# chkda/pytorch-distributed-tutorials

Hardware: AMD Instinct MI355X
Metric: images/sec (whole node) ResNet-50 bf16 at 1/2/4/8 MI355X (higher is better)
Workload: dtype bf16; 1 GPU; model=resnet50, global_batch=256, image_size=224, parallelism=dp1, impl=native, backend=nccl, wire_dtype=fp32, comm_backend=auto, cudnn_benchmark=False, graph=False, deterministic=False, force_comm=False, plan_world=1

## Files before the change

build_native.py:

```python
#!/usr/bin/env python3
from __future__ import annotations

import argparse
import concurrent.futures as cf
import glob
import os
import shlex
import subprocess
import sys
import sysconfig

ROOT = os.path.dirname(os.path.abspath(__file__))
CSRC = os.path.join(ROOT, "csrc")
PKG = os.path.join(ROOT, "pytorch_distributed_tutorials_amd")
BUILD = os.path.join(ROOT, "build", "native")
ARCH = os.environ.get("PYTORCH_ROCM_ARCH", "gfx950").split(";")[0]
HIPCC = os.environ.get("HIPCC", "/opt/rocm/bin/hipcc")


def _torch_paths():
    import torch
    tdir = os.path.dirname(torch.__file__)
    inc = [os.path.join(tdir, "include"), os.path.join(tdir, "include", "torch", "csrc", "api", "include")]
    return tdir, inc, int(torch._C._GLIBCXX_USE_CXX11_ABI)
# ... 67 lines not shown
    os.makedirs(os.path.dirname(so), exist_ok=True)
    if force or jobs_list or not os.path.exists(so) or os.path.getmtime(so) < max(os.path.getmtime(o) for o in objs):
        tlib = os.path.join(tdir, "lib")
        link = [HIPCC, "-shared", "-fPIC", f"--offload-arch={ARCH}", "-o", so] + objs + [
            "-L", tlib, "-lc10", "-lc10_hip", "-ltorch", "-ltorch_cpu", "-ltorch_hip", "-ltorch_python",
            os.path.join(tlib, "librccl.so"), f"-Wl,-rpath,{tlib}", "-Wl,-rpath,/opt/rocm/lib"]
        if sanitize:
            link += ["-fsanitize=address,undefined", "-shared-libsan"]
        _run(link)
        if verbose:
            print(f"[build_native] linked {os.path.relpath(so, ROOT)}", flush=True)
    return so


def ensure_built(verbose: bool = False) -> str:
    return build(force=False, verbose=verbose)


def main(argv=None) -> int:
    ap = argparse.ArgumentParser(description=__doc__, formatter_class=argparse.RawDescriptionHelpFormatter)
    ap.add_argument("--force", action="store_true")
    ap.add_argument("--jobs", type=int, default=0)
    ap.add_argument("--debug", action="store_true")
    ap.add_argument("--sanitize", action="store_true", help="host ASan+UBSan build into build/asan/")
    a = ap.parse_args(argv)
    so = build(force=a.force, jobs=a.jobs, debug=a.debug, sanitize=a.sanitize)
    print(so)
    return 0


# ... 3 lines not shown
```

csrc/bindings.cpp:

```cpp
#include <ATen/ATen.h>
#include <c10/hip/HIPGuard.h>
#include <c10/hip/HIPCachingAllocator.h>
#include <c10/hip/HIPStream.h>
#include <torch/extension.h>

#include <cstdlib>
#include <optional>
#include <stdexcept>
#include <string>
#include <type_traits>
#include <unordered_map>

#include "comm/rccl_comm.h"
#include "comm/xgmi_comm.h"
#include "ddp/reducer.h"
#include "kernels/kernels.h"

namespace py = pybind11;
using at::Tensor;

namespace {

bool g_sync_check = [] {
  const char* e = std::getenv("PDT_SYNC_CHECK");
// ... 310 lines not shown
  TORCH_CHECK(stats.numel() == 4 * K && gamma.numel() == K && sums.numel() == 2 * K && sums.is_contiguous(),
              "BN operands: [4,K], [K], [2,K]");
  int* dp = nullptr;
  if (done.has_value() && done->defined()) {
    TORCH_CHECK(done->is_cuda() && done->scalar_type() == at::kInt && done->numel() >= C / 64 + 1,
                "done: int32 device counters [C / 64 + 1]");
    dp = done->data_ptr<int>();
  }
  TORCH_CHECK(!zero_sums || dp != nullptr, "zero_sums needs the completion counter");
  c10::hip::HIPGuard g(wt.get_device());
  auto pg = bn_param_sinks(dgamma, dbeta, K);
  pdt::launch_bn_fold_wgrad(t1.data_ptr<float>(), gram.data_ptr<float>(), colsum.data_ptr<float>(),
                            reinterpret_cast<const uint16_t*>(wt.data_ptr()), stats.data_ptr<float>(),
                            gamma.data_ptr<float>(), sums.data_ptr<float>(), (int)count, C, K, out.data_ptr<float>(),
                            pg.first, pg.second, dp, zero_sums, cur_stream(wt), csum_slots);
}

std::tuple<Tensor, Tensor> conv_dgrad_bn_fold(const Tensor& g, const Tensor& z_in, const Tensor& wfold,
                                              const Tensor& bias, const Tensor& y, const std::optional<Tensor>& z,
                                              const Tensor& stats, int64_t mask, const std::optional<Tensor>& acc,
                                              const std::optional<Tensor>& dgamma,
                                              const std::optional<Tensor>& dbeta) {
  check_bf16_nhwc(g, "g");
  check_bf16_nhwc(z_in, "z_in");
  const int K = g.size(3), C = z_in.size(3);
  TORCH_CHECK(z_in.size(0) == g.size(0) && z_in.size(1) == g.size(1) && z_in.size(2) == g.size(2),
              "fold: g and z must share N, H, W");
  TORCH_CHECK(wfold.scalar_type() == at::kBFloat16 && wfold.is_contiguous() && wfold.size(0) == C &&
              wfold.size(1) == K + C, "wfold must be bf16 [C][K + C]");
  TORCH_CHECK(bias.scalar_type() == at::kFloat && bias.numel() == C, "bias: fp32 [C]");
// ... 1143 lines not shown
  m.def("stem_bwd_fused", checked("stem_bwd_fused", &stem_bwd_fused), py::arg("dpool"), py::arg("idx"),
        py::arg("y"), py::arg("stats"), py::arg("gamma"), py::arg("sums"), py::arg("training"), py::arg("xsp"),
        py::arg("w_shape"), py::arg("deterministic") = false, py::arg("out") = py::none());
  m.def("stem_bwd_fused_supported", &pdt::stem_bwd_fused_supported, py::arg("K"), py::arg("R"), py::arg("Sp"),
        py::arg("Ho"), py::arg("Wo"));
  m.def("bn_finalize", checked("bn_finalize", &bn_finalize), py::arg("part"), py::arg("count"), py::arg("rm"),
        py::arg("rv"), py::arg("gamma"), py::arg("beta"), py::arg("momentum"), py::arg("eps"),
        py::arg("grows") = 0);
  m.def("bn_eval_params", checked("bn_eval_params", &bn_eval_params));
  m.def("bn_fold_weights", checked("bn_fold_weights", &bn_fold_weights), py::arg("wt"), py::arg("stats"),
        py::arg("gamma"), py::arg("sums"), py::arg("count"));
  m.def("bn_fold_wgrad", checked("bn_fold_wgrad", &bn_fold_wgrad), py::arg("t1"), py::arg("gram"),
        py::arg("colsum"), py::arg("wt"), py::arg("stats"), py::arg("gamma"), py::arg("sums"), py::arg("count"),
        py::arg("out"), py::arg("dgamma") = py::none(), py::arg("dbeta") = py::none(),
        py::arg("done") = py::none(), py::arg("zero_sums") = false);
  m.def("conv_dgrad_bn_fold", checked("conv_dgrad_bn_fold", &conv_dgrad_bn_fold), py::arg("g"), py::arg("z_in"),
        py::arg("wfold"), py::arg("bias"), py::arg("y"), py::arg("z"), py::arg("stats"), py::arg("mask"),
        py::arg("acc") = py::none(), py::arg("dgamma") = py::none(), py::arg("dbeta") = py::none());
  m.def("conv_fwd_bn", checked("conv_fwd_bn", &conv_fwd_bn), py::arg("x"), py::arg("wk"), py::arg("stride"),
        py::arg("pad"), py::arg("count"), py::arg("rm"), py::arg("rv"), py::arg("gamma"), py::arg("beta"),
        py::arg("momentum"), py::arg("eps"), py::arg("acc") = py::none());
  m.def("bn_act_fwd", checked("bn_act_fwd", &bn_act_fwd), py::arg("y"), py::arg("scale"), py::arg("shift"),
        py::arg("residual"), py::arg("relu"), py::arg("res_scale") = py::none(),
        py::arg("res_shift") = py::none(), py::arg("csum") = py::none());
  m.def("bn_act_fwd_mask", checked("bn_act_fwd_mask", &bn_act_fwd_mask), py::arg("y"), py::arg("scale"),
        py::arg("shift"), py::arg("residual"), py::arg("res_scale") = py::none(),
        py::arg("res_shift") = py::none());
  m.def("bn_act_bwd_reduce", checked("bn_act_bwd_reduce", &bn_act_bwd_reduce), py::arg("dz"), py::arg("z"), py::arg("y"),
        py::arg("stats"), py::arg("mask"), py::arg("dgamma") = py::none(), py::arg("dbeta") = py::none());
  m.def("bn_act_bwd_apply", checked("bn_act_bwd_apply", &bn_act_bwd_apply), py::arg("dz"), py::arg("z"),
// ... 91 lines not shown
  m.def("conv_wgrad_cu_reserve", &pdt::conv_wgrad_cu_reserve);
  m.def("conv_wgrad_plan", [](std::vector<int64_t> x_shape, std::vector<int64_t> w_shape, int stride, int pad,
                              bool deterministic) {
    TORCH_CHECK(x_shape.size() == 4 && w_shape.size() == 4, "x_shape [N,H,W,C], w_shape [K,C,R,S]");
    pdt::ConvShape s{};
    s.N = (int)x_shape[0]; s.H = (int)x_shape[1]; s.W = (int)x_shape[2]; s.C = (int)x_shape[3];
    s.K = (int)w_shape[0]; s.R = (int)w_shape[2]; s.S = (int)w_shape[3];
    s.stride = stride; s.pad = pad;
    s.Ho = (s.H + 2 * pad - s.R) / stride + 1; s.Wo = (s.W + 2 * pad - s.S) / stride + 1;
    int out[4];
    pdt::conv_wgrad_plan(s, deterministic, out);
    py::dict d;
    d["bm"] = out[0]; d["bn"] = out[1]; d["tiles"] = out[2]; d["splits"] = out[3];
    return d;
  }, py::arg("x_shape"), py::arg("w_shape"), py::arg("stride"), py::arg("pad"), py::arg("deterministic") = false);
  m.def("bn_counter_bank", [](uintptr_t stream) {
    return pdt::bn_counter_bank(reinterpret_cast<hipStream_t>(stream));
  }, py::arg("stream"));
  m.def("cu_masked_stream", [](int device, int ncu) {
    c10::hip::HIPGuard guard((c10::DeviceIndex)device);
    int total = 0;
    if (hipDeviceGetAttribute(&total, hipDeviceAttributeMultiprocessorCount, device) != hipSuccess || total <= 0)
      throw std::runtime_error("cu_masked_stream: cannot query the CU count");
    ncu = std::max(1, std::min(ncu, total));
    std::vector<uint32_t> mask((total + 31) / 32, 0u);
    for (int i = 0; i < ncu; ++i) {
      const int cu = (int)((int64_t)i * total / ncu);
      mask[cu / 32] |= 1u << (cu % 32);
    }
    hipStream_t s = nullptr;
// ... 114 lines not shown
```

csrc/kernels/bn_act.hip:

```cpp
#include "common.h"
#include "fp8_util.h"
#include "igemm_common.h"
#include "kernels.h"
#include "pool_quad.h"

#include <algorithm>
#include <cstdlib>
#include <mutex>
#include <numeric>
#include <stdexcept>
#include <unordered_map>

namespace pdt {

__device__ __forceinline__ void load8(const float* p, float (&v)[8]) {
  float4 a = *reinterpret_cast<const float4*>(p);
  float4 b = *reinterpret_cast<const float4*>(p + 4);
  v[0] = a.x; v[1] = a.y; v[2] = a.z; v[3] = a.w; v[4] = b.x; v[5] = b.y; v[6] = b.z; v[7] = b.w;
}

#ifndef PDT_FIN_CH
#define PDT_FIN_CH 32
#endif
constexpr int FIN_CH = PDT_FIN_CH;
// ... 216 lines not shown
    a = -k1 * k2;
    b = -k1 * (sums[k] * invM - mu * k2);
  }
};

constexpr int kFoldMaxK = 2048;
constexpr int kCsumSlots = 128, kCsumBlocks = 4096;
typedef __bf16 fold_v8bf __attribute__((ext_vector_type(8)));

__global__ void __launch_bounds__(256) bn_fold_coef_kernel(FoldCoef cf, float* __restrict__ coef) {
  __builtin_amdgcn_s_setprio(3);
  const int k = blockIdx.x * 256 + threadIdx.x;
  if (k < cf.K) cf.ab(k, coef[k], coef[cf.K + k]);
}

__global__ void __launch_bounds__(256) bn_fold_weights_kernel(const uint16_t* __restrict__ wt, FoldCoef cf,
                                                              const float* __restrict__ coef, int C, int nG,
                                                              uint16_t* __restrict__ wfold,
                                                              float* __restrict__ bias,
                                                              float* __restrict__ part) {
  __builtin_amdgcn_s_setprio(3);
  const int K = cf.K, t = threadIdx.x;
  const int KC = K + C;
  const int bid = blockIdx.x;
  if (bid >= nG) {
    const int64_t e = ((int64_t)(bid - nG) * 256 + t) * 8;
    if (e >= (int64_t)C * K) return;
    const int c = (int)(e / K), k = (int)(e - (int64_t)c * K);
    f8 v = unpack8(*reinterpret_cast<const uint4*>(wt + e));
    float g8[8], i8[8];
// ... 24 lines not shown
    xa[q] = *reinterpret_cast<const uint4*>(pa + q * 16);
    xb[q] = *reinterpret_cast<const uint4*>(pb + q * 16);
  }
  for (int k0 = 0; k0 < kq; k0 += 16 * B4) {
    const bool more = k0 + 16 * B4 < kq;
    if (more) {
#pragma unroll
      for (int q = 0; q < B4; ++q) {
        ya[q] = *reinterpret_cast<const uint4*>(pa + k0 + 16 * B4 + q * 16);
        yb[q] = *reinterpret_cast<const uint4*>(pb + k0 + 16 * B4 + q * 16);
      }
    }
#pragma unroll
    for (int q = 0; q < B4; ++q) {
      const int kb = k0 + q * 16;
      float a8[8];
      load8(ca_ + kb, a8);
      f8 fa = unpack8(xa[q]);
      if (with_bias) {
        float b8[8];
        load8(cb_ + kb, b8);
#pragma unroll
        for (int e = 0; e < 8; ++e) bacc = fmaf(fa.v[e], b8[e], bacc);
      }
#pragma unroll
      for (int e = 0; e < 8; ++e) fa.v[e] *= a8[e];
      const uint4 qa = pack8(fa);
      acc = __builtin_amdgcn_mfma_f32_32x32x16_bf16(__builtin_bit_cast(fold_v8bf, qa),
                                                    __builtin_bit_cast(fold_v8bf, xb[q]), acc, 0, 0, 0);
    }
    if (more) {
#pragma unroll
      for (int q = 0; q < B4; ++q) { xa[q] = ya[q]; xb[q] = yb[q]; }
    }
  }
  float* pw = part + (size_t)bid * (3 * 17 * 64);
// ... 130 lines not shown
}

void launch_bn_fold_wgrad(float* t1, float* gram, const float* colsum, const uint16_t* wt,
                          const float* stats, const float* gamma, const float* sums, int M, int C, int K,
                          float* out, float* dgamma, float* dbeta, int* done, bool zero_sums, hipStream_t st,
                          int csum_slots) {
  if (C % kFoldTile != 0 || K % kFoldTile != 0)
    throw std::runtime_error("bn_fold_wgrad: needs C % 64 == 0, K % 64 == 0");
  if (csum_slots != 1 && (csum_slots != kCsumSlots || done == nullptr))
    throw std::runtime_error("bn_fold_wgrad: column sums come as 1 vector, or bn_act_fwd's slots in consume mode");
  FoldCoef cf{stats, gamma, sums, K, 1.f / (float)M};
  hipLaunchKernelGGL(bn_fold_wgrad_kernel, dim3((K / kFoldTile) * (C / kFoldTile)), dim3(256), 0, st, t1, gram,
                     colsum, wt, cf, C, out, dgamma, dbeta, done, zero_sums ? 1 : 0, csum_slots);
}

int64_t bn_fold_weights_ws_floats(int C, int K) { return C + 2 * (int64_t)K + (int64_t)(C / 32) * (C / 32) * 3 * 17 * 64; }

void launch_bn_fold_weights(const uint16_t* wt, const float* stats, const float* gamma, const float* sums,
                            int M, int C, int K, uint16_t* wfold, float* bias, hipStream_t st) {
  if (C % 32 != 0 || K % 256 != 0 || K > kFoldMaxK)
    throw std::runtime_error("bn_fold_weights: needs C % 32 == 0, K % 256 == 0, K <= 2048");
  const int nG = (C / 32) * (C / 32);
  const int nS = (int)(((int64_t)C * K / 8 + 255) / 256);
  FoldCoef cf{stats, gamma, sums, K, 1.f / (float)M};
  float* coef = bias + C;
  float* part = coef + 2 * K;
  hipLaunchKernelGGL(bn_fold_coef_kernel, dim3(ceil_div(K, 256)), dim3(256), 0, st, cf, coef);
  hipLaunchKernelGGL(bn_fold_weights_kernel, dim3(nG + nS), dim3(256), 0, st, wt, cf, coef, C, nG, wfold, bias,
                     part);
}

__global__ void bn_eval_params_kernel(const float* rm, const float* rv, const float* gamma,
                                      const float* beta, float eps, int K, float* out) {
  int k = blockIdx.x * blockDim.x + threadIdx.x;
  if (k >= K) return;
  float invstd = rsqrtf(rv[k] + eps);
  float sc = gamma[k] * invstd;
  out[k] = rm[k];
  out[K + k] = invstd;
  out[2 * K + k] = sc;
  out[3 * K + k] = beta[k] - rm[k] * sc;
}

void launch_bn_eval_params(const float* rm, const float* rv, const float* gamma, const float* beta,
// ... 761 lines not shown
```

csrc/kernels/kernels.h:

```cpp
#pragma once
#include <hip/hip_runtime.h>
#include <stdint.h>

namespace pdt {

void launch_image_to_nhwc(const float* x, uint16_t* y, int N, int C, int H, int W, int Cp,
                          hipStream_t st);
void launch_pack_weight(const float* w, const int64_t* strides, uint16_t* out, int K, int C,
                        int R, int S, int Cp, hipStream_t st);
void launch_pack_t_batched(const uint16_t* src, uint16_t* dst, const void* table, int ntensors,
                           int max_tiles, hipStream_t st);
size_t pack_t_entry_bytes();
void launch_stem_image(const float* x, uint16_t* xsp, int N, int C, int H, int W, int pad, int Hp,
                       int Wsp, hipStream_t st);
bool stem_halo_supported(int K, int R, int Sp, int Wo);
void launch_stem_conv_fwd(const uint16_t* xsp, const uint16_t* wsp, uint16_t* y, float* part, int N, int Hp,
                          int Wsp, int Ho, int Wo, hipStream_t st);
bool stem_bwd_fused_supported(int K, int R, int Sp, int Ho, int Wo);
int stem_bwd_fused_blocks(int N, int Ho);
void launch_stem_bwd_fused(const uint16_t* dpool, const uint8_t* idx, const uint16_t* y, const float* stats,
                           const float* gamma, const float* sums, bool training, const uint16_t* xsp, int N,
                           int Ho, int Wo, int Hp, int Wsp, float* dwsp, float* ws, hipStream_t st);
void launch_stem_pack_weight(const float* w, const int64_t* strides, uint16_t* wsp, int K, int C,
                             int R, int S, int Sp, hipStream_t st);
// ... 39 lines not shown
  float* acc2 = nullptr;
};
int conv_dgrad_bn_groups(const ConvShape& s, int elem_bytes = 2);
struct DgradFold {
  const uint16_t* a2;
  int CA2;
  const float* bias;
};
int64_t bn_fold_weights_ws_floats(int C, int K);
void launch_bn_fold_weights(const uint16_t* wt, const float* stats, const float* gamma, const float* sums,
                            int M, int C, int K, uint16_t* wfold, float* bias, hipStream_t st);
void launch_bn_fold_wgrad(float* t1, float* gram, const float* colsum, const uint16_t* wt,
                          const float* stats, const float* gamma, const float* sums, int M, int C, int K,
                          float* out, float* dgamma, float* dbeta, int* done, bool zero_sums, hipStream_t st,
                          int csum_slots = 1);
void launch_conv_dgrad(const uint16_t* dy, const uint16_t* wt, uint16_t* dx, const uint16_t* addend,
                       const ConvShape& s, hipStream_t st, const BnBwdFuse* bn = nullptr,
                       int addend_sub = 0, const DgradFold* fold = nullptr);
size_t conv_wgrad_ws_floats(const ConvShape& s, bool deterministic);
void conv_wgrad_plan(const ConvShape& s, bool deterministic, int out[4]);
void conv_wgrad_set_cu_reserve(int n);
int conv_wgrad_cu_reserve();
void conv_wgrad_fp8_plan(const ConvShape& s, int out[4]);
void launch_conv_wgrad_fp8(const uint8_t* dy8, const uint8_t* x8, const float* dy_deq, const float* x_deq,
                           float* dw, const ConvShape& s, bool accumulate, hipStream_t st);
void launch_conv_wgrad(const uint16_t* dy, const uint16_t* x, float* dw, float* ws,
                       const ConvShape& s, bool deterministic, bool accumulate, hipStream_t st,
                       float* zero = nullptr, int zero_n = 0);

int bn_finalize_partitions(int ngroups);
// ... 138 lines not shown
```

csrc/kernels/wgrad.hip:

```cpp
#include "common.h"
#include "igemm_common.h"
#include "kernels.h"

#include <algorithm>
#include <cstdio>
#include <cstdlib>
#include <stdexcept>
#include <string>

namespace pdt {

struct WgArgs {
  const uint16_t* dy;
  const uint16_t* x;
  float* out;
  uint32_t dy_bytes, x_bytes;
  int Mred, Kout, Ncols;
  int H, W, C, S, stride, pad, stride_w;
  FastDiv div_hw, div_w;
  int HoWo, Wo, Ho;
  int steps_per_split, nsteps;
  int adv_r, adv_qh, adv_qn;
  int mode;
  int64_t slab_stride;
  float* zero;
  int zero_n;
};

constexpr int WG_ATOMIC = 0, WG_STORE = 1, WG_ACCUM = 2;

template <int WM, int WN>
struct WgCfg {
  static_assert(WM * WN == 4, "four 64x64 accumulator tiles per block");
  static constexpr int NT = 512;
  static constexpr int BM = WM * 64, BN = WN * 64;
  static constexpr int A_ROWB = BM * 2, B_ROWB = BN * 2;
  static constexpr int A_BYTES = 64 * A_ROWB, B_BYTES = 64 * B_ROWB;
  static constexpr int STAGE = A_BYTES + B_BYTES;
#ifndef PDT_WG_STAGES
#define PDT_WG_STAGES 4
#endif
  static constexpr int STAGES = PDT_WG_STAGES;
  static constexpr int SMEM = STAGES * STAGE;
  static_assert(SMEM <= 163840, "LDS");
  static constexpr int A_LPR = A_ROWB / 16, A_RPI = 64 / A_LPR;
  static constexpr int B_LPR = B_ROWB / 16, B_RPI = 64 / B_LPR;
  static constexpr int A_PW = A_BYTES / 1024 / 8;
  static constexpr int B_PW = B_BYTES / 1024 / 8;
  static_assert(A_PW * 8192 == A_BYTES && B_PW * 8192 == B_BYTES, "tile DMA split");
};

template <int WM, int WN, bool PW>
__global__ void __launch_bounds__(512, 2) wgrad_kernel(const WgArgs P) {
  using CFG = WgCfg<WM, WN>;
  constexpr int A_PW = CFG::A_PW, B_PW = CFG::B_PW, ST = CFG::STAGES;
  constexpr int LPS = A_PW + B_PW;
  extern __shared__ __attribute__((aligned(16))) char smem[];
  if (P.zero != nullptr && blockIdx.x == 0)
    for (int i = threadIdx.x; i < P.zero_n; i += blockDim.x) P.zero[i] = 0.f;

  const int ntn = (P.Ncols + CFG::BN - 1) / CFG::BN;
  const int ntm = (P.Kout + CFG::BM - 1) / CFG::BM;
  const int tiles = ntm * ntn;
  const int lid = xcd_remap(blockIdx.x, gridDim.x);
  const int split = lid / tiles;
  const int bid = lid - split * tiles;
  const int tmi = bid / ntn, tni = bid - tmi * ntn;
  const int k0 = tmi * CFG::BM, c0 = tni * CFG::BN;
  const int s_begin = split * P.steps_per_split;
  const int s_end = min(P.nsteps, s_begin + P.steps_per_split);

  const int t = threadIdx.x;
  const int lane = t & 63, wid = __builtin_amdgcn_readfirstlane(t >> 6);
  const v4i rdy = rsrc_words(P.dy, P.dy_bytes);
  const v4i rx = rsrc_words(P.x, P.x_bytes);
  const uint32_t sbase = lds_addr(smem);

  int a_lane[A_PW];
#pragma unroll
  for (int i = 0; i < A_PW; ++i) {
    const int arow = (wid * A_PW + i) * CFG::A_RPI + lane / CFG::A_LPR;
    const int slot = lane % CFG::A_LPR;
    const int chk = (swz_img<CFG::A_ROWB>(arow, slot) - arow * CFG::A_ROWB) >> 4;
    const int acol = k0 + chk * 8;
    a_lane[i] = acol < P.Kout ? (arow * P.Kout + acol) * 2 : (int)OOB;
  }
  int brow[B_PW], b_dh[B_PW], b_dw[B_PW], b_chb[B_PW];
#pragma unroll
  for (int i = 0; i < B_PW; ++i) {
    brow[i] = (wid * B_PW + i) * CFG::B_RPI + lane / CFG::B_LPR;
    const int slot = lane % CFG::B_LPR;
    const int chk = (swz_img<CFG::B_ROWB>(brow[i], slot) - brow[i] * CFG::B_ROWB) >> 4;
    const int col = c0 + chk * 8;
    const int tap = col / P.C;
    b_chb[i] = col < P.Ncols ? (col - tap * P.C) * 2 : (int)OOB;
    const int r = tap / P.S;
    b_dh[i] = r - P.pad;
    b_dw[i] = (tap - r * P.S) - P.pad;
  }
  const int WC2 = P.W * P.C * 2, HWC2 = P.H * WC2, C2 = P.C * 2;
// ... 1 lines not shown
  if constexpr (!PW) {
#pragma unroll
    for (int i = 0; i < B_PW; ++i) {
      const uint32_t m = (uint32_t)(s_begin * 64 + brow[i]);
      b_n[i] = fdiv(m, P.div_hw);
      const uint32_t rem = m - b_n[i] * (uint32_t)P.HoWo;
      b_ho[i] = fdiv(rem, P.div_w);
      b_wo[i] = rem - b_ho[i] * (uint32_t)P.Wo;
    }
  }

  auto issue = [&](int step, int buf) {
    const uint32_t As = sbase + buf * CFG::STAGE;
    const uint32_t Bs = As + CFG::A_BYTES;
    const int mb = step * 64;
    const int abase = mb * P.Kout * 2;
#pragma unroll
    for (int i = 0; i < A_PW; ++i)
      glds16_asm(rdy, As + (wid * A_PW + i) * 1024, (uint32_t)(abase + a_lane[i]));
#pragma unroll
    for (int i = 0; i < B_PW; ++i) {
      uint32_t off;
      if constexpr (PW) {
        off = (uint32_t)((mb + brow[i]) * C2 + b_chb[i]);
      } else {
        const uint32_t h = __umul24(b_ho[i], (uint32_t)P.stride) + (uint32_t)b_dh[i];
        const uint32_t w = __umul24(b_wo[i], (uint32_t)P.stride_w) + (uint32_t)b_dw[i];
        const bool ok = h < (uint32_t)P.H && w < (uint32_t)P.W;
        const uint32_t o = __umul24(b_n[i], (uint32_t)HWC2) + __umul24(h, (uint32_t)WC2) +
                           __umul24(w, (uint32_t)C2) + (uint32_t)b_chb[i];
        off = ok ? o : OOB;
// ... 97 lines not shown
  __syncthreads();

  const int fq = lane >> 4, fr = lane & 15;
  float* stg = xch + wid * 2048;
#pragma unroll
  for (int ii = 0; ii < 2; ++ii)
#pragma unroll
    for (int jj = 0; jj < 4; ++jj)
#pragma unroll
      for (int e = 0; e < 4; ++e) {
        const int r = ii * 16 + fq * 4 + e;
        stg[r * 64 + ((jj * 16 + fr) ^ (((r >> 2) & 1) << 4))] = acc[keep + ii][jj][e];
      }
  __builtin_amdgcn_s_waitcnt(0xc07f);
  __builtin_amdgcn_wave_barrier();
  float* o = P.out + split * P.slab_stride;
  const int col = c0 + wn * 64 + lane;
  const int row0 = k0 + wm * 64 + keep * 16;
  if (col < P.Ncols) {
#pragma unroll 8
    for (int r = 0; r < 32; ++r) {
      const float v = stg[r * 64 + (lane ^ (((r >> 2) & 1) << 4))];
      if (row0 + r < P.Kout) {
        float* dst = o + (int64_t)(row0 + r) * P.Ncols + col;
        if (P.mode == WG_ATOMIC) unsafeAtomicAdd(dst, v);
        else if (P.mode == WG_ACCUM) *dst += v;
        else *dst = v;
      }
    }
  }
}


struct WhArgs {
  const uint16_t* dy;
  const uint16_t* x;
  float* out;
  uint32_t dy_bytes, x_bytes;
// ... 377 lines not shown
  if (p.slab) {
    const int64_t dw_bytes = (int64_t)s.K * ncols * 4;
    splits = (int)std::min<int64_t>(splits, std::max<int64_t>(1, ((int64_t)64 << 20) / dw_bytes));
  }
  p.steps_per_split = (p.nsteps + splits - 1) / splits;
  p.splits = (p.nsteps + p.steps_per_split - 1) / p.steps_per_split;
  if (p.splits <= 1) p.slab = false;
  return p;
}

void conv_wgrad_plan(const ConvShape& s, bool deterministic, int out[4]) {
  const WgPlan p = plan_wg(s, deterministic);
  out[0] = p.bm; out[1] = p.bn; out[2] = p.tiles; out[3] = p.splits;
}

size_t conv_wgrad_ws_floats(const ConvShape& s, bool deterministic) {
  const WgPlan p = plan_wg(s, deterministic);
  if (!p.slab) return 0;
  return (size_t)p.splits * s.K * s.R * s.S * s.C;
}

template <int WM, int WN, bool PW>
static void run_wg(const WgArgs& a, int nb, hipStream_t st) {
  using CFG = WgCfg<WM, WN>;
  auto kfn = wgrad_kernel<WM, WN, PW>;
  static bool attr_set = false;
  if (!attr_set) {
    hipFuncSetAttribute((const void*)kfn, hipFuncAttributeMaxDynamicSharedMemorySize, CFG::SMEM);
    attr_set = true;
  }
  hipLaunchKernelGGL(kfn, dim3(nb), dim3(CFG::NT), CFG::SMEM, st, a);
  wg_check("wgrad_kernel");
}

template <int WM, int WC, int TC>
static void run_wh(const WhArgs& a, int nb, hipStream_t st) {
  using CFG = WhCfg<WM, WC, TC>;
  auto kfn = wgrad_halo3_kernel<WM, WC, TC>;
  static bool attr_set = false;
  if (!attr_set) {
// ... 59 lines not shown
                    s.H == s.Ho && s.W == s.Wo;
    if (p.wm == 2) { if (pw) run_wg<2, 2, true>(a, nb, st); else run_wg<2, 2, false>(a, nb, st); }
    else if (p.wm == 1) { if (pw) run_wg<1, 4, true>(a, nb, st); else run_wg<1, 4, false>(a, nb, st); }
    else { if (pw) run_wg<4, 1, true>(a, nb, st); else run_wg<4, 1, false>(a, nb, st); }
  }
  if (slab) {
    if (n % 4 != 0) throw std::runtime_error("conv_wgrad: dW size must be a multiple of 4 floats");
    const int64_t n4 = n / 4;
    hipLaunchKernelGGL(wg_splitk_reduce_kernel, dim3((unsigned)((n4 + 15) / 16)), dim3(256), 0, st,
                       reinterpret_cast<const float4*>(ws), p.splits, n4, reinterpret_cast<float4*>(dw),
                       accumulate ? 1 : 0);
    wg_check("splitk_reduce");
  }
}

}
```

pytorch_distributed_tutorials_amd/ops/fused.py:

```python
from __future__ import annotations

import os
import weakref
from typing import Optional

import torch
import torch.nn as nn

from . import reference as ref
from . import streams
from ..utils.seed import deterministic
from ._ext import native

_CPU_DTYPE = torch.float32
_FUSE_DGRAD_BN = True
_BN_HANDOFF = True
_ZMASK = True
_NAN_TRACE = os.environ.get("PDT_NAN_TRACE", "0") == "1"
_FP8 = False
_FP8_BWD = True
_FP8_WGRAD = True
_FP8_ONLY = True
_BN_ACC = True

# ... 977 lines not shown
                dy, dres, d8 = apply(5 * i, dz, z, y, stt, sums, mask, tr, last, need_dx, in8[i] if in8 else None,
                                     st)
            else:
                g, sums = pre
                dres = g
            fold = None
            if pre is not None and _fold_ok(i, last, w, xin, st, pd, tr, det, side, ctx.fp8b, params):
                wt = _packed_crsk(w)
                if wt is None:
                    wt = C.pack_weight_t(w)
                global FOLD_CALLS
                FOLD_CALLS += 1
                k_, c_ = w.shape[0], w.shape[1]
                count = y.numel() // k_
                fold = C.bn_fold_weights(wt.view(c_, k_), stt, gamma, sums, count)
                streams.fork(side, g, stt, sums, wt, xin)
                with torch.cuda.stream(side):
                    t1, gram, done = _fold_ws(k_, c_, xin.device)
                    C.conv_wgrad(g, xin, [k_, c_, 1, 1], 1, 0, det, t1)
                    C.conv_wgrad(xin, xin, [c_, c_, 1, 1], 1, 0, det, gram)
                    colsum = ctx.colsum
                    if colsum is None:
                        colsum = C.bn_act_bwd_reduce(xin, xin, xin, _zero_stats(c_, xin.device), 0)[0]
                    ctx.colsum = None
                    dfr = deferred.pop(5 * i, None)
                    C.bn_fold_wgrad(t1, gram, colsum, wt.view(c_, k_), stt, gamma, sums, count,
                                    _grad_sink(params[5 * i]), dfr[1] if dfr is not None else None,
                                    dfr[2] if dfr is not None else None, done, dfr is not None)
                sunk.append(params[5 * i])
            elif pre is not None:
                dy, _, d8 = apply(5 * i, g, g, y, stt, sums, 0, tr, False, need_dx, in8[i] if in8 else None, st)
            pre = None
            if fold is None:
                wgrad(5 * i, dy, xin, st, pd, d8, in8[i] if in8 else None)
            if last:
                g_short = dres
                if ds_cfg is not None and nch > 1 and ds_br is not None:
                    main = streams.fork(ds_br, g_short, y_ds, st_ds, x)
                    with torch.cuda.stream(ds_br):
                        addend_br = shortcut_backward(g_short)
                    ds_join = (main, streams.join(ds_br, main, addend_br), addend_br)
            if i > 0:
                yp, sttp = units[i - 1][1], units[i - 1][2]
# ... 45 lines not shown
                        dz = dgrad(dy, d8, w, list(x.shape), st, pd, addend)
        ctx.handoff_in = None
        for acc_, _, _ in deferred.values():
            acc_.zero_()
        if ctx.colsum is not None:
            if ctx.colsum.dim() == 2:
                ctx.colsum.zero_()
            ctx.colsum = None
        if sunk:
            sunk[0]._pdt_flat.mark_ready(sunk)
        return (dz, None, None, None, *grads)


_FOLD_BN = True
FOLD_CALLS = 0


def _fold_ok(i, last, w, xin, st, pd, tr, det, side, fp8b, params) -> bool:
    if not (_FOLD_BN and last and i > 0 and tr and side is not None and not fp8b and _BN_ACC
            and _FUSE_DGRAD_BN and xin is not None):
        return False
    k, c, r, s_ = w.shape
    if r != 1 or s_ != 1 or st != 1 or pd != 0 or k % 256 or k > 2048 or c % 64 or xin.shape[3] != c:
        return False
    j = 5 * (i - 1)
    return (_grad_sink(params[j + 1]) is not None and _grad_sink(params[j + 2]) is not None
            and _grad_sink(params[5 * i]) is not None)


def _fold_colsum_ok(chain, tensors, x) -> bool:
# ... 14 lines not shown
    if cs is None or cs.shape[1] != c or cs.device != dev:
        cs = torch.zeros(native().bn_csum_slots(), c, dtype=torch.float32, device=dev)
        w._pdt_csum = cs
    return cs


_ZSTATS = {}
_FOLD_WS = {}


def _fold_ws(k, c, dev):
    ws = _FOLD_WS.get((k, c, dev))
    if ws is None:
        ws = _FOLD_WS[(k, c, dev)] = (torch.zeros(k, c, 1, 1, device=dev), torch.zeros(c, c, 1, 1, device=dev),
                                      torch.zeros(c // 64 + 1, dtype=torch.int32, device=dev))
    return ws


def _zero_stats(c, dev):
    z = _ZSTATS.get((c, dev))
    if z is None:
        z = _ZSTATS[(c, dev)] = torch.zeros(4, c, device=dev)
    return z


def _grad_sink(p):
    sp = getattr(p, "_pdt_flat", None)
    if sp is None or not p.requires_grad or not p.is_cuda:
        return None
    return sp.grad_sink(p)
# ... 32 lines not shown
```

Baseline: 14360 images/sec.

## Merge BN-fold wgrad and gram GEMMs into one kernel with MFMA finish

Replaces the two separate wgrad launches (dy^T·x and x^T·x) in the BN-folded backward path with a single merged wgrad kernel. Its extra tiles compute the gram matrix, and the gamma*invstd scaling is applied directly when writing into the weight-gradient sink. A new finish kernel uses bf16 MFMA with a three-way hi/mid/lo split of the fp32 gram to add the correction term, which drops the t1 intermediate buffer and extra launches. It also adds an optional env-gated inline-coefficient path for bn_fold_weights and a faster ensure_built check. The cost is more complex counters and zeroing logic, plus possible precision differences from the bf16 split.

Measured after the change: 14490 images/sec, median of 6. About the same (+0.9%).

```diff
diff --git a/build_native.py b/build_native.py
--- a/build_native.py
+++ b/build_native.py
@@ -105,6 +105,11 @@
 
 
 def ensure_built(verbose: bool = False) -> str:
+    so = out_path()
+    if os.path.exists(so):
+        srcs = [p for pat in ("**/*.hip", "**/*.cpp", "**/*.h") for p in glob.glob(os.path.join(CSRC, pat), recursive=True)]
+        if srcs and os.path.getmtime(so) >= max(os.path.getmtime(p) for p in srcs):
+            return so
     return build(force=False, verbose=verbose)
 
 
diff --git a/csrc/bindings.cpp b/csrc/bindings.cpp
--- a/csrc/bindings.cpp
+++ b/csrc/bindings.cpp
@@ -348,6 +348,66 @@
                             reinterpret_cast<const uint16_t*>(wt.data_ptr()), stats.data_ptr<float>(),
                             gamma.data_ptr<float>(), sums.data_ptr<float>(), (int)count, C, K, out.data_ptr<float>(),
                             pg.first, pg.second, dp, zero_sums, cur_stream(wt), csum_slots);
+}
+
+static void check_kc_dense(const Tensor& t, int64_t rows, int64_t cols, const char* what) {
+  TORCH_CHECK(t.is_cuda() && t.scalar_type() == at::kFloat && t.numel() == rows * cols && t.dim() >= 2 &&
+              t.size(0) == rows && t.size(1) == cols && t.stride(0) == cols && t.stride(1) == 1,
+              what, ": fp32 device [", rows, "][", cols, "]-dense");
+}
+
+void conv_wgrad_fold(const Tensor& g, const Tensor& x, const Tensor& stats, const Tensor& gamma, Tensor out,
+                     Tensor gram) {
+  check_cuda(g, "g");
+  check_cuda(x, "x");
+  TORCH_CHECK(g.scalar_type() == at::kBFloat16 && x.scalar_type() == at::kBFloat16 && g.dim() == 4 && x.dim() == 4 &&
+              g.is_contiguous() && x.is_contiguous(), "conv_wgrad_fold: g, x must be contiguous bf16 [N,H,W,*]");
+  TORCH_CHECK(g.size(0) == x.size(0) && g.size(1) == x.size(1) && g.size(2) == x.size(2),
+              "conv_wgrad_fold: g and x must share N, H, W");
+  const int64_t K = g.size(3), C = x.size(3), M = g.numel() / K;
+  TORCH_CHECK(M > 0 && M < ((int64_t)1 << 30), "conv_wgrad_fold: row count out of range");
+  TORCH_CHECK(stats.is_cuda() && stats.scalar_type() == at::kFloat && stats.is_contiguous() && stats.numel() == 4 * K,
+              "stats: fp32 [4, K]");
+  TORCH_CHECK(gamma.is_cuda() && gamma.scalar_type() == at::kFloat && gamma.is_contiguous() && gamma.numel() == K,
+              "gamma: fp32 [K]");
+  check_kc_dense(out, K, C, "out");
+  check_kc_dense(gram, C, C, "gram");
+  c10::hip::HIPGuard guard(g.get_device());
+  pdt::launch_conv_wgrad_fold(cbf(g), cbf(x), out.data_ptr<float>(), gram.data_ptr<float>(), gamma.data_ptr<float>(),
+                              stats.data_ptr<float>(), (int)M, (int)C, (int)K, cur_stream(g));
+}
+
+void bn_fold_finish(Tensor gram, const Tensor& colsum, const Tensor& w, const Tensor& stats, const Tensor& gamma,
+                    const Tensor& sums, int64_t count, Tensor out, const std::optional<Tensor>& dgamma,
+                    const std::optional<Tensor>& dbeta, const std::optional<Tensor>& done, bool zero_sums) {
+  check_cuda(w, "w");
+  check_cuda(colsum, "colsum");
+  TORCH_CHECK(w.scalar_type() == at::kBFloat16 && w.is_contiguous() && w.numel() == w.size(0) * w.size(-1),
+              "w must be contiguous bf16 [K][C]");
+  const int K = w.size(0), C = w.size(-1);
+  const int S = pdt::bn_csum_slots();
+  TORCH_CHECK(colsum.scalar_type() == at::kFloat && colsum.is_contiguous() &&
+              (colsum.numel() == C || (colsum.dim() == 2 && colsum.size(0) == S && colsum.size(1) == C)),
+              "colsum: fp32 [C] or [bn_csum_slots(), C]");
+  const int csum_slots = colsum.dim() == 2 ? S : 1;
+  check_kc_dense(out, K, C, "out");
+  check_kc_dense(gram, C, C, "gram");
+  TORCH_CHECK(stats.is_cuda() && gamma.is_cuda() && sums.is_cuda() && stats.scalar_type() == at::kFloat &&
+              gamma.scalar_type() == at::kFloat && sums.scalar_type() == at::kFloat && stats.is_contiguous() &&
+              gamma.is_contiguous() && stats.numel() == 4 * K && gamma.numel() == K && sums.numel() == 2 * K &&
+              sums.is_contiguous(), "BN operands: fp32 [4,K], [K], [2,K]");
+  int* dp = nullptr;
+  if (done.has_value() && done->defined()) {
+    TORCH_CHECK(done->is_cuda() && done->scalar_type() == at::kInt && done->is_contiguous() &&
+                done->numel() >= C / 32 + 1, "done: int32 device counters [C / 32 + 1]");
+    dp = done->data_ptr<int>();
+  }
+  TORCH_CHECK(!zero_sums || dp != nullptr, "zero_sums needs the completion counter");
+  c10::hip::HIPGuard guard(w.get_device());
+  auto pg = bn_param_sinks(dgamma, dbeta, K);
+  pdt::launch_bn_fold_finish(gram.data_ptr<float>(), colsum.data_ptr<float>(), cbf(w), stats.data_ptr<float>(),
+                             gamma.data_ptr<float>(), sums.data_ptr<float>(), (int)count, C, K, out.data_ptr<float>(),
+                             pg.first, pg.second, dp, zero_sums, cur_stream(w), csum_slots);
 }
 
 std::tuple<Tensor, Tensor> conv_dgrad_bn_fold(const Tensor& g, const Tensor& z_in, const Tensor& wfold,
@@ -1521,6 +1581,12 @@
         py::arg("colsum"), py::arg("wt"), py::arg("stats"), py::arg("gamma"), py::arg("sums"), py::arg("count"),
         py::arg("out"), py::arg("dgamma") = py::none(), py::arg("dbeta") = py::none(),
         py::arg("done") = py::none(), py::arg("zero_sums") = false);
+  m.def("conv_wgrad_fold", checked("conv_wgrad_fold", &conv_wgrad_fold), py::arg("g"), py::arg("x"),
+        py::arg("stats"), py::arg("gamma"), py::arg("out"), py::arg("gram"));
+  m.def("bn_fold_finish", checked("bn_fold_finish", &bn_fold_finish), py::arg("gram"), py::arg("colsum"),
+        py::arg("w"), py::arg("stats"), py::arg("gamma"), py::arg("sums"), py::arg("count"), py::arg("out"),
+        py::arg("dgamma") = py::none(), py::arg("dbeta") = py::none(), py::arg("done") = py::none(),
+        py::arg("zero_sums") = false);
   m.def("conv_dgrad_bn_fold", checked("conv_dgrad_bn_fold", &conv_dgrad_bn_fold), py::arg("g"), py::arg("z_in"),
         py::arg("wfold"), py::arg("bias"), py::arg("y"), py::arg("z"), py::arg("stats"), py::arg("mask"),
         py::arg("acc") = py::none(), py::arg("dgamma") = py::none(), py::arg("dbeta") = py::none());
@@ -1642,6 +1708,14 @@
     d["bm"] = out[0]; d["bn"] = out[1]; d["tiles"] = out[2]; d["splits"] = out[3];
     return d;
   }, py::arg("x_shape"), py::arg("w_shape"), py::arg("stride"), py::arg("pad"), py::arg("deterministic") = false);
+  m.def("conv_wgrad_fold_plan", [](int64_t M, int64_t C, int64_t K) {
+    TORCH_CHECK(M > 0 && M < ((int64_t)1 << 30) && C > 0 && K > 0, "conv_wgrad_fold_plan: M rows, C, K channels");
+    int out[4];
+    pdt::conv_wgrad_fold_plan((int)M, (int)C, (int)K, out);
+    py::dict d;
+    d["bm"] = out[0]; d["bn"] = out[1]; d["tiles"] = out[2]; d["splits"] = out[3];
+    return d;
+  }, py::arg("M"), py::arg("C"), py::arg("K"));
   m.def("bn_counter_bank", [](uintptr_t stream) {
     return pdt::bn_counter_bank(reinterpret_cast<hipStream_t>(stream));
   }, py::arg("stream"));
diff --git a/csrc/kernels/bn_act.hip b/csrc/kernels/bn_act.hip
--- a/csrc/kernels/bn_act.hip
+++ b/csrc/kernels/bn_act.hip
@@ -254,6 +254,7 @@
   if (k < cf.K) cf.ab(k, coef[k], coef[cf.K + k]);
 }
 
+template <bool INL>
 __global__ void __launch_bounds__(256) bn_fold_weights_kernel(const uint16_t* __restrict__ wt, FoldCoef cf,
                                                               const float* __restrict__ coef, int C, int nG,
                                                               uint16_t* __restrict__ wfold,
@@ -308,12 +309,33 @@
 #pragma unroll
     for (int q = 0; q < B4; ++q) {
       const int kb = k0 + q * 16;
-      float a8[8];
-      load8(ca_ + kb, a8);
+      float a8[8], b8[8];
+      if constexpr (INL) {
+        const int k = kbeg + kh + kb;
+        float is8[8], g8[8], s18[8];
+        load8(cf.stats + K + k, is8);
+        load8(cf.gamma + k, g8);
+        load8(cf.sums + K + k, s18);
+        float k18[8], k28[8];
+#pragma unroll
+        for (int e = 0; e < 8; ++e) {
+          k18[e] = g8[e] * is8[e];
+          k28[e] = s18[e] * is8[e] * is8[e] * cf.invM;
+          a8[e] = -k18[e] * k28[e];
+        }
+        if (with_bias) {
+          float mu8[8], s08[8];
+          load8(cf.stats + k, mu8);
+          load8(cf.sums + k, s08);
+#pragma unroll
+          for (int e = 0; e < 8; ++e) b8[e] = -k18[e] * (s08[e] * cf.invM - mu8[e] * k28[e]);
+        }
+      } else {
+        load8(ca_ + kb, a8);
+        if (with_bias) load8(cb_ + kb, b8);
+      }
       f8 fa = unpack8(xa[q]);
       if (with_bias) {
-        float b8[8];
-        load8(cb_ + kb, b8);
 #pragma unroll
         for (int e = 0; e < 8; ++e) bacc = fmaf(fa.v[e], b8[e], bacc);
       }
@@ -474,6 +496,138 @@
                      colsum, wt, cf, C, out, dgamma, dbeta, done, zero_sums ? 1 : 0, csum_slots);
 }
 
+__device__ __forceinline__ void fold_split3(const float v, uint32_t& h, uint32_t& m, uint32_t& l) {
+  h = __float_as_uint(v) & 0xffff0000u;
+  const float r1 = v - __uint_as_float(h);
+  m = __float_as_uint(r1) & 0xffff0000u;
+  const float r2 = r1 - __uint_as_float(m);
+  l = __float_as_uint(r2) & 0xffff0000u;
+}
+
+template <int BQ>
+__global__ void __launch_bounds__(256) bn_fold_finish_kernel(float* __restrict__ gram,
+                                                             const float* __restrict__ colsum,
+                                                             const uint16_t* __restrict__ w, FoldCoef cf, int C,
+                                                             float* __restrict__ out, float* __restrict__ dgamma,
+                                                             float* __restrict__ dbeta, int* __restrict__ done,
+                                                             int zero_sums, int csum_slots) {
+  const int K = cf.K, t = threadIdx.x;
+  const int nc = C / 32;
+  const int tk = blockIdx.x / nc, tc = blockIdx.x - tk * nc;
+  const int k0 = tk * 32, c0 = tc * 32;
+  if (blockIdx.x == 0 && dgamma != nullptr) {
+    for (int k = t; k < K; k += 256) {
+      const float is = cf.stats[K + k];
+      dgamma[k] += cf.sums[K + k] * is;
+      dbeta[k] += cf.sums[k];
+    }
+  }
+  const int wv = t >> 6, lane = t & 63;
+  const int r = lane & 31, hf = lane >> 5;
+  const int qn = C / 4, qbeg = wv * qn;
+  const uint16_t* pa = w + (size_t)(k0 + r) * C + qbeg + hf * 8;
+  const float* pg = gram + (size_t)(c0 + r) * C + qbeg + hf * 8;
+  uint4 xa[BQ], ya[BQ];
+  float4 g0[BQ], g1[BQ], h0[BQ], h1[BQ];
+#pragma unroll
+  for (int q = 0; q < BQ; ++q) {
+    xa[q] = *reinterpret_cast<const uint4*>(pa + q * 16);
+    g0[q] = *reinterpret_cast<const float4*>(pg + q * 16);
+    g1[q] = *reinterpret_cast<const float4*>(pg + q * 16 + 4);
+  }
+  float ca, cb;
+  cf.ab(k0 + r, ca, cb);
+  float cs = 0.f;
+#pragma unroll 8
+  for (int sl = wv * 2 + hf; sl < csum_slots; sl += 8) cs += colsum[(size_t)sl * C + c0 + r];
+  cs += __shfl_xor(cs, 32, 64);
+  v16f acc = {};
+  for (int q0 = 0; q0 < qn; q0 += 16 * BQ) {
+    const bool more = q0 + 16 * BQ < qn;
+    if (more) {
+#pragma unroll
+      for (int q = 0; q < BQ; ++q) {
+        ya[q] = *reinterpret_cast<const uint4*>(pa + q0 + 16 * BQ + q * 16);
+        h0[q] = *reinterpret_cast<const float4*>(pg + q0 + 16 * BQ + q * 16);
+        h1[q] = *reinterpret_cast<const float4*>(pg + q0 + 16 * BQ + q * 16 + 4);
+      }
+    }
+#pragma unroll
+    for (int q = 0; q < BQ; ++q) {
+      const float gv[8] = {g0[q].x, g0[q].y, g0[q].z, g0[q].w, g1[q].x, g1[q].y, g1[q].z, g1[q].w};
+      uint32_t ph[4], pm[4], pl[4];
+#pragma unroll
+      for (int e = 0; e < 4; ++e) {
+        uint32_t ha, ma, la, hb, mb, lb;
+        fold_split3(gv[2 * e], ha, ma, la);
+        fold_split3(gv[2 * e + 1], hb, mb, lb);
+        ph[e] = (ha >> 16) | hb;
+        pm[e] = (ma >> 16) | mb;
+        pl[e] = (la >> 16) | lb;
+      }
+      const fold_v8bf fa = __builtin_bit_cast(fold_v8bf, xa[q]);
+      acc = __builtin_amdgcn_mfma_f32_32x32x16_bf16(fa, __builtin_bit_cast(fold_v8bf, make_uint4(pl[0], pl[1], pl[2], pl[3])), acc, 0, 0, 0);
+      acc = __builtin_amdgcn_mfma_f32_32x32x16_bf16(fa, __builtin_bit_cast(fold_v8bf, make_uint4(pm[0], pm[1], pm[2], pm[3])), acc, 0, 0, 0);
+      acc = __builtin_amdgcn_mfma_f32_32x32x16_bf16(fa, __builtin_bit_cast(fold_v8bf, make_uint4(ph[0], ph[1], ph[2], ph[3])), acc, 0, 0, 0);
+    }
+    if (more) {
+#pragma unroll
+      for (int q = 0; q < BQ; ++q) { xa[q] = ya[q]; g0[q] = h0[q]; g1[q] = h1[q]; }
+    }
+  }
+#pragma unroll
+  for (int e = 0; e < 16; ++e) {
+    const int row = 8 * (e >> 2) + 4 * hf + (e & 3);
+    const float a = __shfl(ca, row, 64), b = __shfl(cb, row, 64);
+    unsafeAtomicAdd(out + (size_t)(k0 + row) * C + c0 + r, a * acc[e] + b * cs);
+  }
+  if (done == nullptr) return;
+  __syncthreads();
+  if (wv != 0) return;
+  int last = 0;
+  if (lane == 0) {
+    __threadfence();
+    const int nk = K / 32;
+    last = atomicAdd(done + tc, 1) == nk - 1 ? 1 : 0;
+    if (last) {
+      done[tc] = 0;
+      __threadfence();
+      last = atomicAdd(done + nc, 1) == nc - 1 ? 2 : 1;
+      if (last == 2) done[nc] = 0;
+    }
+  }
+  last = __shfl(last, 0, 64);
+  if (last == 0) return;
+  __threadfence();
+  float4* grow = reinterpret_cast<float4*>(gram + (size_t)c0 * C);
+  for (int e = lane; e < 8 * C; e += 64) grow[e] = make_float4(0.f, 0.f, 0.f, 0.f);
+  if (csum_slots > 1)
+    for (int e = lane; e < csum_slots * 32; e += 64)
+      const_cast<float*>(colsum)[(size_t)(e >> 5) * C + c0 + (e & 31)] = 0.f;
+  if (last == 2 && zero_sums) {
+    float* sm = const_cast<float*>(cf.sums);
+    for (int e = lane; e < 2 * K; e += 64) sm[e] = 0.f;
+  }
+}
+
+void launch_bn_fold_finish(float* gram, const float* colsum, const uint16_t* w, const float* stats,
+                           const float* gamma, const float* sums, int M, int C, int K, float* out, float* dgamma,
+                           float* dbeta, int* done, bool zero_sums, hipStream_t st, int csum_slots) {
+  if (C % 64 != 0 || K % 32 != 0) throw std::runtime_error("bn_fold_finish: needs C % 64 == 0, K % 32 == 0");
+  if (csum_slots != 1 && (csum_slots != kCsumSlots || done == nullptr))
+    throw std::runtime_error("bn_fold_finish: column sums come as 1 vector, or bn_act_fwd's slots in consume mode");
+  FoldCoef cf{stats, gamma, sums, K, 1.f / (float)M};
+  const dim3 grid((K / 32) * (C / 32));
+  const int ns = C / 64;
+#define PDT_FOLD_FINISH(BQ)                                                                                    \
+  hipLaunchKernelGGL(bn_fold_finish_kernel<BQ>, grid, dim3(256), 0, st, gram, colsum, w, cf, C, out, dgamma, \
+                     dbeta, done, zero_sums ? 1 : 0, csum_slots)
+  if (ns % 4 == 0) PDT_FOLD_FINISH(4);
+  else if (ns % 2 == 0) PDT_FOLD_FINISH(2);
+  else PDT_FOLD_FINISH(1);
+#undef PDT_FOLD_FINISH
+}
+
 int64_t bn_fold_weights_ws_floats(int C, int K) { return C + 2 * (int64_t)K + (int64_t)(C / 32) * (C / 32) * 3 * 17 * 64; }
 
 void launch_bn_fold_weights(const uint16_t* wt, const float* stats, const float* gamma, const float* sums,
@@ -485,9 +639,18 @@
   FoldCoef cf{stats, gamma, sums, K, 1.f / (float)M};
   float* coef = bias + C;
   float* part = coef + 2 * K;
+  static const bool inl = [] {
+    const char* e = std::getenv("PDT_FOLD_COEF_INLINE");
+    return e != nullptr && e[0] == '1';
+  }();
+  if (inl) {
+    hipLaunchKernelGGL(bn_fold_weights_kernel<true>, dim3(nG + nS), dim3(256), 0, st, wt, cf, coef, C, nG, wfold,
+                       bias, part);
+    return;
+  }
   hipLaunchKernelGGL(bn_fold_coef_kernel, dim3(ceil_div(K, 256)), dim3(256), 0, st, cf, coef);
-  hipLaunchKernelGGL(bn_fold_weights_kernel, dim3(nG + nS), dim3(256), 0, st, wt, cf, coef, C, nG, wfold, bias,
-                     part);
+  hipLaunchKernelGGL(bn_fold_weights_kernel<false>, dim3(nG + nS), dim3(256), 0, st, wt, cf, coef, C, nG, wfold,
+                     bias, part);
 }
 
 __global__ void bn_eval_params_kernel(const float* rm, const float* rv, const float* gamma,
diff --git a/csrc/kernels/kernels.h b/csrc/kernels/kernels.h
--- a/csrc/kernels/kernels.h
+++ b/csrc/kernels/kernels.h
@@ -77,6 +77,12 @@
                           const float* stats, const float* gamma, const float* sums, int M, int C, int K,
                           float* out, float* dgamma, float* dbeta, int* done, bool zero_sums, hipStream_t st,
                           int csum_slots = 1);
+void conv_wgrad_fold_plan(int M, int C, int K, int out[4]);
+void launch_conv_wgrad_fold(const uint16_t* g, const uint16_t* x, float* out, float* gram, const float* gamma,
+                            const float* stats, int M, int C, int K, hipStream_t st);
+void launch_bn_fold_finish(float* gram, const float* colsum, const uint16_t* w, const float* stats,
+                           const float* gamma, const float* sums, int M, int C, int K, float* out, float* dgamma,
+                           float* dbeta, int* done, bool zero_sums, hipStream_t st, int csum_slots = 1);
 void launch_conv_dgrad(const uint16_t* dy, const uint16_t* wt, uint16_t* dx, const uint16_t* addend,
                        const ConvShape& s, hipStream_t st, const BnBwdFuse* bn = nullptr,
                        int addend_sub = 0, const DgradFold* fold = nullptr);
diff --git a/csrc/kernels/wgrad.hip b/csrc/kernels/wgrad.hip
--- a/csrc/kernels/wgrad.hip
+++ b/csrc/kernels/wgrad.hip
@@ -25,6 +25,9 @@
   int64_t slab_stride;
   float* zero;
   int zero_n;
+  float* gram;
+  const float* fold_gamma;
+  const float* fold_stats;
 };
 
 constexpr int WG_ATOMIC = 0, WG_STORE = 1, WG_ACCUM = 2;
@@ -50,8 +53,9 @@
   static_assert(A_PW * 8192 == A_BYTES && B_PW * 8192 == B_BYTES, "tile DMA split");
 };
 
-template <int WM, int WN, bool PW>
+template <int WM, int WN, bool PW, bool FOLD = false>
 __global__ void __launch_bounds__(512, 2) wgrad_kernel(const WgArgs P) {
+  static_assert(PW || !FOLD, "fold mode is pointwise");
   using CFG = WgCfg<WM, WN>;
   constexpr int A_PW = CFG::A_PW, B_PW = CFG::B_PW, ST = CFG::STAGES;
   constexpr int LPS = A_PW + B_PW;
@@ -60,20 +64,28 @@
     for (int i = threadIdx.x; i < P.zero_n; i += blockDim.x) P.zero[i] = 0.f;
 
   const int ntn = (P.Ncols + CFG::BN - 1) / CFG::BN;
-  const int ntm = (P.Kout + CFG::BM - 1) / CFG::BM;
+  const int ntm_g = (P.Kout + CFG::BM - 1) / CFG::BM;
+  const int ntm = FOLD ? ntm_g + (P.C + CFG::BM - 1) / CFG::BM : ntm_g;
   const int tiles = ntm * ntn;
   const int lid = xcd_remap(blockIdx.x, gridDim.x);
   const int split = lid / tiles;
   const int bid = lid - split * tiles;
-  const int tmi = bid / ntn, tni = bid - tmi * ntn;
+  int tmi = bid / ntn;
+  const int tni = bid - tmi * ntn;
+  int kout = P.Kout;
+  bool gram_tile = false;
+  if constexpr (FOLD) {
+    gram_tile = tmi >= ntm_g;
+    if (gram_tile) { tmi -= ntm_g; kout = P.C; }
+  }
   const int k0 = tmi * CFG::BM, c0 = tni * CFG::BN;
   const int s_begin = split * P.steps_per_split;
   const int s_end = min(P.nsteps, s_begin + P.steps_per_split);
 
   const int t = threadIdx.x;
   const int lane = t & 63, wid = __builtin_amdgcn_readfirstlane(t >> 6);
-  const v4i rdy = rsrc_words(P.dy, P.dy_bytes);
   const v4i rx = rsrc_words(P.x, P.x_bytes);
+  const v4i rdy = (FOLD && gram_tile) ? rx : rsrc_words(P.dy, P.dy_bytes);
   const uint32_t sbase = lds_addr(smem);
 
   int a_lane[A_PW];
@@ -83,7 +95,7 @@
     const int slot = lane % CFG::A_LPR;
     const int chk = (swz_img<CFG::A_ROWB>(arow, slot) - arow * CFG::A_ROWB) >> 4;
     const int acol = k0 + chk * 8;
-    a_lane[i] = acol < P.Kout ? (arow * P.Kout + acol) * 2 : (int)OOB;
+    a_lane[i] = acol < kout ? (arow * kout + acol) * 2 : (int)OOB;
   }
   int brow[B_PW], b_dh[B_PW], b_dw[B_PW], b_chb[B_PW];
 #pragma unroll
@@ -115,7 +127,7 @@
     const uint32_t As = sbase + buf * CFG::STAGE;
     const uint32_t Bs = As + CFG::A_BYTES;
     const int mb = step * 64;
-    const int abase = mb * P.Kout * 2;
+    const int abase = mb * kout * 2;
 #pragma unroll
     for (int i = 0; i < A_PW; ++i)
       glds16_asm(rdy, As + (wid * A_PW + i) * 1024, (uint32_t)(abase + a_lane[i]));
@@ -243,14 +255,16 @@
       }
   __builtin_amdgcn_s_waitcnt(0xc07f);
   __builtin_amdgcn_wave_barrier();
-  float* o = P.out + split * P.slab_stride;
+  float* o = (FOLD && gram_tile) ? P.gram : P.out + split * P.slab_stride;
   const int col = c0 + wn * 64 + lane;
   const int row0 = k0 + wm * 64 + keep * 16;
   if (col < P.Ncols) {
 #pragma unroll 8
     for (int r = 0; r < 32; ++r) {
-      const float v = stg[r * 64 + (lane ^ (((r >> 2) & 1) << 4))];
-      if (row0 + r < P.Kout) {
+      float v = stg[r * 64 + (lane ^ (((r >> 2) & 1) << 4))];
+      if (row0 + r < kout) {
+        if constexpr (FOLD)
+          if (!gram_tile) v *= P.fold_gamma[row0 + r] * P.fold_stats[P.Kout + row0 + r];
         float* dst = o + (int64_t)(row0 + r) * P.Ncols + col;
         if (P.mode == WG_ATOMIC) unsafeAtomicAdd(dst, v);
         else if (P.mode == WG_ACCUM) *dst += v;
@@ -658,16 +672,38 @@
   out[0] = p.bm; out[1] = p.bn; out[2] = p.tiles; out[3] = p.splits;
 }
 
+static WgPlan plan_wg_fold(int M, int C, int K) {
+  WgPlan p{};
+  p.kind = KIND_GEN;
+  if (C <= 64 && K % 256 == 0) { p.wm = 4; p.wn = 1; }
+  else { p.wm = 2; p.wn = 2; }
+  p.bm = p.wm * 64; p.bn = p.wn * 64;
+  p.tiles = ((K + p.bm - 1) / p.bm + (C + p.bm - 1) / p.bm) * ((C + p.bn - 1) / p.bn);
+  p.nsteps = (M + 63) / 64;
+  const double mfma_cyc = (double)p.bm * p.bn * 64 * 2 / 4096.0;
+  const double t_step = std::max(mfma_cyc * 2.0 / 2400.0, 64.0 * (p.bm + p.bn) * 2 / 50.0e3);
+  double est_us = 0.0;
+  const int splits = choose_splits(p.tiles, p.nsteps, t_step, (double)p.bm * p.bn * 4, false, &est_us);
+  p.steps_per_split = (p.nsteps + splits - 1) / splits;
+  p.splits = (p.nsteps + p.steps_per_split - 1) / p.steps_per_split;
+  return p;
+}
+
+void conv_wgrad_fold_plan(int M, int C, int K, int out[4]) {
+  const WgPlan p = plan_wg_fold(M, C, K);
+  out[0] = p.bm; out[1] = p.bn; out[2] = p.tiles; out[3] = p.splits;
+}
+
 size_t conv_wgrad_ws_floats(const ConvShape& s, bool deterministic) {
   const WgPlan p = plan_wg(s, deterministic);
   if (!p.slab) return 0;
   return (size_t)p.splits * s.K * s.R * s.S * s.C;
 }
 
-template <int WM, int WN, bool PW>
+template <int WM, int WN, bool PW, bool FOLD = false>
 static void run_wg(const WgArgs& a, int nb, hipStream_t st) {
   using CFG = WgCfg<WM, WN>;
-  auto kfn = wgrad_kernel<WM, WN, PW>;
+  auto kfn = wgrad_kernel<WM, WN, PW, FOLD>;
   static bool attr_set = false;
   if (!attr_set) {
     hipFuncSetAttribute((const void*)kfn, hipFuncAttributeMaxDynamicSharedMemorySize, CFG::SMEM);
@@ -757,4 +793,30 @@
   }
 }
 
-}
+void launch_conv_wgrad_fold(const uint16_t* g, const uint16_t* x, float* out, float* gram, const float* gamma,
+                            const float* stats, int M, int C, int K, hipStream_t st) {
+  if (C % 8 != 0 || K % 8 != 0) throw std::runtime_error("conv_wgrad_fold: channels must be multiples of 8");
+  if ((int64_t)M * K * 2 >= ((int64_t)1 << 31) || M <= 0)
+    throw std::runtime_error("conv_wgrad_fold: g must be smaller than 2 GB");
+  const WgPlan p = plan_wg_fold(M, C, K);
+  WgArgs a{};
+  a.dy = g; a.x = x; a.out = out; a.gram = gram;
+  a.fold_gamma = gamma; a.fold_stats = stats;
+  a.dy_bytes = (uint32_t)((int64_t)M * K * 2);
+  a.x_bytes = (uint32_t)((int64_t)M * C * 2);
+  a.Mred = M; a.Kout = K; a.Ncols = C;
+  a.H = 1; a.W = M; a.C = C; a.S = 1; a.stride = 1; a.pad = 0; a.stride_w = 1;
+  a.HoWo = M; a.Wo = M; a.Ho = 1;
+  a.div_hw = make_fastdiv((uint32_t)M);
+  a.div_w = make_fastdiv((uint32_t)M);
+  a.steps_per_split = p.steps_per_split;
+  a.nsteps = p.nsteps;
+  a.mode = p.splits > 1 ? WG_ATOMIC : WG_ACCUM;
+  a.slab_stride = 0;
+  a.zero = nullptr; a.zero_n = 0;
+  const int nb = p.tiles * p.splits;
+  if (p.wm == 4) run_wg<4, 1, true, true>(a, nb, st);
+  else run_wg<2, 2, true, true>(a, nb, st);
+}
+
+}
diff --git a/pytorch_distributed_tutorials_amd/ops/fused.py b/pytorch_distributed_tutorials_amd/ops/fused.py
--- a/pytorch_distributed_tutorials_amd/ops/fused.py
+++ b/pytorch_distributed_tutorials_amd/ops/fused.py
@@ -1015,19 +1015,28 @@
                 k_, c_ = w.shape[0], w.shape[1]
                 count = y.numel() // k_
                 fold = C.bn_fold_weights(wt.view(c_, k_), stt, gamma, sums, count)
-                streams.fork(side, g, stt, sums, wt, xin)
+                merged = _FOLD_MERGED and not det
+                wk = _packed_krsc(C, w, c_) if merged else None
+                streams.fork(side, g, stt, sums, wt, xin, wk)
                 with torch.cuda.stream(side):
-                    t1, gram, done = _fold_ws(k_, c_, xin.device)
-                    C.conv_wgrad(g, xin, [k_, c_, 1, 1], 1, 0, det, t1)
-                    C.conv_wgrad(xin, xin, [c_, c_, 1, 1], 1, 0, det, gram)
                     colsum = ctx.colsum
                     if colsum is None:
                         colsum = C.bn_act_bwd_reduce(xin, xin, xin, _zero_stats(c_, xin.device), 0)[0]
                     ctx.colsum = None
                     dfr = deferred.pop(5 * i, None)
-                    C.bn_fold_wgrad(t1, gram, colsum, wt.view(c_, k_), stt, gamma, sums, count,
-                                    _grad_sink(params[5 * i]), dfr[1] if dfr is not None else None,
-                                    dfr[2] if dfr is not None else None, done, dfr is not None)
+                    sink = _grad_sink(params[5 * i])
+                    dg, db = (dfr[1], dfr[2]) if dfr is not None else (None, None)
+                    if merged:
+                        gram, done = _fold_ws_merged(c_, xin.device)
+                        C.conv_wgrad_fold(g, xin, stt, gamma, sink, gram)
+                        C.bn_fold_finish(gram, colsum, wk.view(k_, c_), stt, gamma, sums, count, sink, dg, db, done,
+                                         dfr is not None)
+                    else:
+                        t1, gram, done = _fold_ws(k_, c_, xin.device)
+                        C.conv_wgrad(g, xin, [k_, c_, 1, 1], 1, 0, det, t1)
+                        C.conv_wgrad(xin, xin, [c_, c_, 1, 1], 1, 0, det, gram)
+                        C.bn_fold_wgrad(t1, gram, colsum, wt.view(c_, k_), stt, gamma, sums, count, sink, dg, db,
+                                        done, dfr is not None)
                 sunk.append(params[5 * i])
             elif pre is not None:
                 dy, _, d8 = apply(5 * i, g, g, y, stt, sums, 0, tr, False, need_dx, in8[i] if in8 else None, st)
@@ -1103,6 +1112,7 @@
 
 _FOLD_BN = True
 FOLD_CALLS = 0
+_FOLD_MERGED = os.environ.get("PDT_FOLD_MERGED", "1") == "1"
 
 
 def _fold_ok(i, last, w, xin, st, pd, tr, det, side, fp8b, params) -> bool:
@@ -1147,6 +1157,17 @@
     if ws is None:
         ws = _FOLD_WS[(k, c, dev)] = (torch.zeros(k, c, 1, 1, device=dev), torch.zeros(c, c, 1, 1, device=dev),
                                       torch.zeros(c // 64 + 1, dtype=torch.int32, device=dev))
+    return ws
+
+
+_FOLD_WS_MERGED = {}
+
+
+def _fold_ws_merged(c, dev):
+    ws = _FOLD_WS_MERGED.get((c, dev))
+    if ws is None:
+        ws = _FOLD_WS_MERGED[(c, dev)] = (torch.zeros(c, c, device=dev),
+                                          torch.zeros(c // 32 + 1, dtype=torch.int32, device=dev))
     return ws
 
 
```
